# PRBonn/RAP

Measured on AMD Instinct MI355X. Metric: registered points/sec @20 flow steps, 2-view N=4096, higher is better.
Workload: dtype f32; 1 GPU; configs[1]: batch=32 samples/GPU x 2 views x 4096 pts, 20 Euler flow steps, rap_12 (d=512, H=8), fp32 (exact-fp32 MFMA), rigidity_forcing=on, final per-view SE(3) fit; preset=1, pairs_per_gpu=32, views=2, points_per_view=4096, flow_steps=20, num_layers=12, rigidity_forcing=True

## Files before the change

### rap_amd/csrc/api.hip

```cpp
#include "../../include/rapflow.h"
#include "half.h"
#include "kernels.h"

#include <mutex>
#include <new>
#include <vector>

static thread_local int g_last_hip_error = 0;
void rap_set_last_hip_error(int e) { g_last_hip_error = e; }

#define RAP_PROF_CLASSES 8
struct ProfRec { hipEvent_t a, b; int cls; };
static std::atomic<bool> g_prof_on{false};
static std::mutex g_prof_mu;
static std::vector<ProfRec> g_prof_recs;
static std::vector<hipEvent_t> g_prof_pool;
static size_t g_prof_pool_used = 0;
static const size_t RAP_PROF_MAX_EVENTS = 1u << 19;

static hipEvent_t prof_event() {
  if (g_prof_pool_used < g_prof_pool.size()) return g_prof_pool[g_prof_pool_used++];
  if (g_prof_pool.size() >= RAP_PROF_MAX_EVENTS) return nullptr;
  hipEvent_t e = nullptr;
  if (hipEventCreate(&e) != hipSuccess) return nullptr;
  g_prof_pool.push_back(e);
  g_prof_pool_used++;
  return e;
}
struct ProfScope {
  hipStream_t s; hipEvent_t a = nullptr, b = nullptr; int cls;
  ProfScope(hipStream_t s_, int cls_) : s(s_), cls(cls_) {
    if (!g_prof_on.load(std::memory_order_relaxed)) return;
    std::lock_guard<std::mutex> lock(g_prof_mu);
    a = prof_event(); b = prof_event();
    if (a && b) (void)hipEventRecord(a, s); else a = b = nullptr;
  }
  ~ProfScope() {
    if (a && b) {
      std::lock_guard<std::mutex> lock(g_prof_mu);
      (void)hipEventRecord(b, s); g_prof_recs.push_back({a, b, cls});
    }
  }
};
extern "C" int rap_profile_enable(int on) { g_prof_on.store(on != 0); return RAP_OK; }
extern "C" int rap_profile_reset(void) { std::lock_guard<std::mutex> lock(g_prof_mu); g_prof_recs.clear(); g_prof_pool_used = 0; return RAP_OK; }
extern "C" int rap_profile_collect_ex(float* h_ms_out, int64_t* h_count_out, int32_t n_classes) {
  if (!h_ms_out || !h_count_out || n_classes <= 0) return RAP_ERR_INVALID;
  std::lock_guard<std::mutex> lock(g_prof_mu);
  for (int c = 0; c < n_classes; ++c) { h_ms_out[c] = 0.f; h_count_out[c] = 0; }
  for (const ProfRec& r : g_prof_recs) {
    if (r.cls >= n_classes) continue;
    if (hipEventSynchronize(r.b) != hipSuccess) return RAP_ERR_HIP;
    float ms = 0.f;
    if (hipEventElapsedTime(&ms, r.a, r.b) != hipSuccess) return RAP_ERR_HIP;
    h_ms_out[r.cls] += ms; h_count_out[r.cls] += 1;
  }
  return RAP_OK;
}
extern "C" int rap_profile_collect(float* h_ms_out, int64_t* h_count_out) { return rap_profile_collect_ex(h_ms_out, h_count_out, 3); }

struct LayerW {
  const float* Wqkv[2];
  const float* Wout[2];
  const float* bout[2];
  const float* gq[2];
  const float* gk[2];
  const float* ffn_g;
  const float* ffn_b;
  const float* Wff1p;
  const float* bff1p;
  const float* Wff2;
  const float* bff2;
};

struct LayerWH {
  const u16* Wqkv[2];
  const u16* Wout[2];
  const u16* Wff1p;
  const u16* Wff2;
  float s_qkv[2] = {1.f, 1.f}, s_out[2] = {1.f, 1.f}, s_ff1 = 1.f, s_ff2 = 1.f;
  float g_v[2] = {1.f, 1.f}, g_ff1 = 1.f;
};
struct HalfWeights {
  u16* blob = nullptr;
  std::vector<LayerWH> layers;
};
#define RAP_MAX_LOGIT_BOUND 40.0f

struct rap_model {
  rap_model_desc desc;
  int d, L, H, F, E;
  int Din = 0;
  int Ks = 128;
  int dtype = RAP_DT_F32;
  bool qk_norm = true;
  int resid_dtype = RAP_DT_F32;
  HalfWeights half[4];
  float* logit_bound = nullptr;
  std::vector<uint8_t> bounded;
  int n_bounded = 0;
  float* raw = nullptr;
  float* derived = nullptr;
  const float* anchor_emb;
  const float* emb_bias;
  const float* Wstatic;
  const float* Wx;
  const float *adaW1, *adab1, *adaW2, *adab2, *adaW3, *adab3;
  std::vector<LayerW> layers;
  const float *hW0, *hb0, *hW2, *hb2, *hW4;
  mutable std::mutex cfg_mu;
};

static bool desc_ok(const rap_model_desc* d) {
  if (!d) return false;
  if (d->embed_dim <= 0 || d->embed_dim % 256 != 0 || d->embed_dim > 1024) return false;
  if (d->num_heads * 64 != d->embed_dim) return false;
  if (d->num_layers <= 0 || d->num_layers > 64) return false;
  if (d->local_feat_dim < 0 || d->local_feat_dim % 4 != 0 || d->local_feat_dim > 40) return false;
  return true;
}

extern rap_tuning_t g_rap_gemm_variant;
extern rap_tuning_t g_rap_gemm_stagger;
extern rap_tuning_t g_rap_gemm_splitk;
extern rap_tuning_t g_rap_geglu_fast;
extern rap_tuning_t g_rap_attn_split;
extern rap_tuning_t g_rap_gemm_h16_variant;
extern rap_tuning_t g_rap_attn_h16_variant;
extern rap_tuning_t g_rap_gemm_h16_persistent;
extern rap_tuning_t g_rap_attn_h16_dma;
extern rap_tuning_t g_rap_gemm_f32_persistent;
extern rap_tuning_t g_rap_attn_x2_wpe;
extern rap_tuning_t g_rap_attn_h16_small;
rap_tuning_t g_rap_attn_lpt = 1;
rap_tuning_t g_rap_x2_min_rows = 1024;
rap_tuning_t g_rap_small_fused = 1;
extern rap_tuning_t g_rap_ring_blocks;
rap_tuning_t g_rap_fuse_qknorm = 1;
struct TuningRow { int32_t key; rap_tuning_t* var; int n_values; int32_t values[7]; };
static const TuningRow kTuning[] = {
#ifdef RAP_ABLATION_BUILD
  {0, &g_rap_gemm_variant, 3, {16, 32, 48}},
  {2, &g_rap_gemm_h16_variant, 3, {0, 1, 14}},
  {3, &g_rap_attn_h16_variant, 2, {0, 5}},
  {4, &g_rap_gemm_stagger, 3, {0, 1, 2}},
#endif
  {5, &g_rap_attn_split, 2, {0, 1}},
  {6, &g_rap_gemm_splitk, 2, {0, 1}},
  {7, &g_rap_fuse_qknorm, 2, {0, 1}},
  {9, &g_rap_geglu_fast, 2, {0, 1}},
  {11, &g_rap_gemm_h16_persistent, 2, {0, 1}},
  {12, &g_rap_gemm_f32_persistent, 2, {0, 1}},
  {13, &g_rap_attn_h16_dma, 2, {0, 1}},
  {15, &g_rap_attn_lpt, 2, {0, 1}},
  {16, &g_rap_attn_x2_wpe, 2, {2, 4}},
  {17, &g_rap_x2_min_rows, -1, {}},
  {18, &g_rap_ring_blocks, -1, {}},
  {19, &g_rap_small_fused, 2, {0, 1}},
  {20, &g_rap_attn_h16_small, 7, {0, 1, 2, 64, 128, 66, 130}},
};
extern "C" int rap_set_tuning(int32_t key, int32_t value) {
  for (const TuningRow& r : kTuning) {
    if (r.key != key) continue;
    bool ok = r.n_values < 0 && value >= 0;
    for (int i = 0; i < r.n_values; ++i) ok = ok || r.values[i] == value;
    if (ok) *r.var = value;
    return ok ? RAP_OK : RAP_ERR_INVALID;
  }
  return RAP_ERR_INVALID;
}

extern "C" int rap_version(void) { return RAPFLOW_ABI_VERSION; }
extern "C" int rap_last_hip_error(void) { return g_last_hip_error; }

static bool in_dim_ok(int32_t in_dim) { return in_dim >= 0 && in_dim <= 512 && in_dim % 4 == 0; }
extern "C" int64_t rap_weight_count(const rap_model_desc* desc) { return rap_weight_count_latent(desc, 0); }
extern "C" int64_t rap_weight_count_latent(const rap_model_desc* desc, int32_t in_dim) {
  if (!desc_ok(desc) || !in_dim_ok(in_dim)) return -1;
  const int64_t d = desc->embed_dim, L = desc->num_layers, H = desc->num_heads, E = 147 + desc->local_feat_dim + in_dim;
  int64_t n = 2 * d + d * E + d;
  const int64_t attn = (d * 256 + d) + (d * d + d) + (2 * d * d + 2 * d) + 3 * d * d + (d * d + d) + 2 * H * 64;
  const int64_t layer = 2 * attn + 2 * d + (8 * d * d + 8 * d) + (4 * d * d + d);
  n += L * layer;
  n += (d * d + d) + (d / 2 * d + d / 2) + 3 * (d / 2);
  return n;
}

static int ensure_logit_bounds(rap_model* m, hipStream_t stream);

extern "C" int rap_model_create(const rap_model_desc* desc, const float* d_weights, int64_t n_floats, void* stream_,
                                rap_model** out) {
  return rap_model_create_latent(desc, 0, d_weights, n_floats, stream_, out);
}
extern "C" int rap_model_create_latent(const rap_model_desc* desc, int32_t in_dim, const float* d_weights, int64_t n_floats, void* stream_,
                                       rap_model** out) {
  if (!out) return RAP_ERR_INVALID;
  *out = nullptr;
  if (!desc_ok(desc) || !in_dim_ok(in_dim) || !d_weights) return RAP_ERR_INVALID;
  if (n_floats != rap_weight_count_latent(desc, in_dim)) return RAP_ERR_INVALID;
  hipStream_t stream = (hipStream_t)stream_;
  rap_model* m = new (std::nothrow) rap_model();
  if (!m) return RAP_ERR_ALLOC;
  m->desc = *desc;
  const int d = m->d = desc->embed_dim, L = m->L = desc->num_layers, H = m->H = desc->num_heads;
  m->F = desc->local_feat_dim;
  m->Din = in_dim;
  const int Ks = m->Ks = 128 + (in_dim + 31) / 32 * 32;
  const int E = m->E = 147 + m->F + m->Din;
  if (hipMalloc((void**)&m->raw, (size_t)n_floats * sizeof(float)) != hipSuccess) { delete m; return RAP_ERR_ALLOC; }
  const size_t n_ada = (size_t)2 * L * ((size_t)d * 256 + d + (size_t)d * d + d + (size_t)2 * d * d + 2 * d);
  const size_t n_ff1 = (size_t)L * ((size_t)8 * d * d + 8 * d);
  const size_t n_derived = (size_t)d * Ks + (size_t)d * 64 + n_ada + n_ff1;
  if (hipMalloc((void**)&m->derived, n_derived * sizeof(float)) != hipSuccess) {
    (void)hipFree(m->raw); delete m; return RAP_ERR_ALLOC;
  }
  int rc = RAP_OK;
  auto fail = [&](int code) { rap_model_destroy(m); return code; };
  if (hipMemcpyAsync(m->raw, d_weights, (size_t)n_floats * sizeof(float), hipMemcpyDeviceToDevice, stream) != hipSuccess)
    return fail(RAP_ERR_HIP);

  const float* p = m->raw;
  auto take = [&](size_t n) { const float* r = p; p += n; return r; };
  m->anchor_emb = take((size_t)2 * d);
  const float* embW = take((size_t)d * E);
  m->emb_bias = take(d);

  float* q = m->derived;
  auto carve = [&](size_t n) { float* r = q; q += n; return r; };
  float* Wstatic = carve((size_t)d * Ks);
  float* Wx = carve((size_t)d * 64);
  float* aW1 = carve((size_t)2 * L * d * 256); float* ab1 = carve((size_t)2 * L * d);
  float* aW2 = carve((size_t)2 * L * d * d);   float* ab2 = carve((size_t)2 * L * d);
  float* aW3 = carve((size_t)2 * L * 2 * d * d); float* ab3 = carve((size_t)2 * L * 2 * d);
  m->Wstatic = Wstatic; m->Wx = Wx;
  m->adaW1 = aW1; m->adab1 = ab1; m->adaW2 = aW2; m->adab2 = ab2; m->adaW3 = aW3; m->adab3 = ab3;

  if ((rc = launch_fill_zero(stream, Wstatic, (size_t)d * Ks))) return fail(rc);
  if ((rc = launch_fill_zero(stream, Wx, (size_t)d * 64))) return fail(rc);
  if ((rc = launch_copy_cols(stream, embW, E, 0, Wstatic, Ks, 0, d, 63))) return fail(rc);
  if ((rc = launch_copy_cols(stream, embW, E, 126, Wstatic, Ks, 63, d, 21))) return fail(rc);
  if ((rc = launch_copy_cols(stream, embW, E, 147, Wstatic, Ks, 84, d, m->F))) return fail(rc);
  if ((rc = launch_copy_cols(stream, embW, E, 147 + m->F, Wstatic, Ks, 128, d, m->Din))) return fail(rc);
  if ((rc = launch_copy_cols(stream, embW, E, 63, Wx, 64, 0, d, 63))) return fail(rc);

  m->layers.resize(L);
  for (int i = 0; i < L; ++i) {
    LayerW& lw = m->layers[i];
    for (int a = 0; a < 2; ++a) {
      const int j = 2 * i + a;
      const float* W1 = take((size_t)d * 256); const float* b1 = take(d);
      const float* W2 = take((size_t)d * d);   const float* b2 = take(d);
      const float* W3 = take((size_t)2 * d * d); const float* b3 = take((size_t)2 * d);
      if ((rc = launch_copy_cols(stream, W1, 256, 0, aW1 + (size_t)j * d * 256, 256, 0, d, 256))) return fail(rc);
      if ((rc = launch_copy_cols(stream, b1, d, 0, ab1 + (size_t)j * d, d, 0, 1, d))) return fail(rc);
      if ((rc = launch_copy_cols(stream, W2, d, 0, aW2 + (size_t)j * d * d, d, 0, d, d))) return fail(rc);
      if ((rc = launch_copy_cols(stream, b2, d, 0, ab2 + (size_t)j * d, d, 0, 1, d))) return fail(rc);
      if ((rc = launch_copy_cols(stream, W3, d, 0, aW3 + (size_t)j * 2 * d * d, d, 0, 2 * d, d))) return fail(rc);
      if ((rc = launch_copy_cols(stream, b3, 2 * d, 0, ab3 + (size_t)j * 2 * d, 2 * d, 0, 1, 2 * d))) return fail(rc);
      lw.Wqkv[a] = take((size_t)3 * d * d);
      lw.Wout[a] = take((size_t)d * d);
      lw.bout[a] = take(d);
      lw.gq[a] = take((size_t)H * 64);
      lw.gk[a] = take((size_t)H * 64);
    }
    lw.ffn_g = take(d);
    lw.ffn_b = take(d);
    const float* Wff1 = take((size_t)8 * d * d);
    const float* bff1 = take((size_t)8 * d);
    float* Wp = carve((size_t)8 * d * d);
    float* bp = carve((size_t)8 * d);
    if ((rc = launch_geglu_interleave(stream, Wff1, bff1, Wp, bp, 4 * d, d))) return fail(rc);
    lw.Wff1p = Wp; lw.bff1p = bp;
    lw.Wff2 = take((size_t)d * 4 * d);
    lw.bff2 = take(d);
  }
  m->hW0 = take((size_t)d * d); m->hb0 = take(d);
  m->hW2 = take((size_t)(d / 2) * d); m->hb2 = take(d / 2);
  m->hW4 = take((size_t)3 * (d / 2));
  if ((int64_t)(p - m->raw) != n_floats || (size_t)(q - m->derived) != n_derived) return fail(RAP_ERR_INVALID);
  if ((rc = ensure_logit_bounds(m, stream))) return fail(rc);
  *out = m;
  return RAP_OK;
}

extern "C" void rap_model_destroy(rap_model* m) {
  if (!m) return;
  if (m->raw) (void)hipFree(m->raw);
  if (m->derived) (void)hipFree(m->derived);
  for (int i = 0; i < 4; ++i)
    if (m->half[i].blob) (void)hipFree(m->half[i].blob);
  if (m->logit_bound) (void)hipFree(m->logit_bound);
  delete m;
}

static int ensure_logit_bounds(rap_model* m, hipStream_t stream) {
  if (m->logit_bound) return RAP_OK;
  const int n = m->L * 2 * m->H;
  if (hipMalloc((void**)&m->logit_bound, (size_t)n * sizeof(float)) != hipSuccess) { m->logit_bound = nullptr; return RAP_ERR_ALLOC; }
  for (int i = 0; i < m->L; ++i)
    for (int a = 0; a < 2; ++a) {
      const int rc = launch_qk_logit_bound(stream, m->layers[i].gq[a], m->layers[i].gk[a], m->H, m->logit_bound + (size_t)(2 * i + a) * m->H);
      if (rc) return rc;
    }
  std::vector<float> hb(n);
  RAP_HIP_CHECK(hipMemcpyAsync(hb.data(), m->logit_bound, (size_t)n * sizeof(float), hipMemcpyDeviceToHost, stream));
  RAP_HIP_CHECK(hipStreamSynchronize(stream));
  m->bounded.assign((size_t)2 * m->L, 1);
  for (int j = 0; j < 2 * m->L; ++j)
    for (int h = 0; h < m->H; ++h)
      if (!(hb[(size_t)j * m->H + h] <= RAP_MAX_LOGIT_BOUND)) m->bounded[j] = 0;
  m->n_bounded = 0;
  for (uint8_t b : m->bounded) m->n_bounded += b;
// ... 600 lines not shown
```

### rap_amd/csrc/attn_f32.hip

```cpp
#include "kernels.h"

#define AQ_WAVE 64
#define AKV 64
#define KLD 68
#define VLD 64
#define ATTN_FENCE __builtin_amdgcn_sched_barrier(0x406);

__device__ __forceinline__ float xhalf_max(float v) {
  const auto r = __builtin_amdgcn_permlane32_swap(__float_as_uint(v), __float_as_uint(v), false, false);
  return fmaxf(__uint_as_float(r[0]), __uint_as_float(r[1]));
}
__device__ __forceinline__ float xhalf_sum(float v) {
  const auto r = __builtin_amdgcn_permlane32_swap(__float_as_uint(v), __float_as_uint(v), false, false);
  return __uint_as_float(r[0]) + __uint_as_float(r[1]);
}

#define ATTN_DEFER_THR 11.5f
__device__ __forceinline__ float amax3(float a, float b, float c) {
  float r;
  asm("v_max3_f32 %0, %1, %2, %3" : "=v"(r) : "v"(a), "v"(b), "v"(c));
  return r;
}

template <int NW, bool BOUNDED, bool SPLIT = false>
__global__ __launch_bounds__(64 * NW, 2) void attention_f32_kernel(const float* __restrict__ qkv, float* __restrict__ out,
                                                                  int TP, int heads, const AttnWorkItem* __restrict__ items,
                                                                  const float* __restrict__ bound, float* __restrict__ part_o,
                                                                  float* __restrict__ part_l) {
  __shared__ __attribute__((aligned(16))) float smem[2 * AKV * KLD + 2 * AKV * VLD];
  float* Ks = smem;
  float* Vs = smem + 2 * AKV * KLD;

  const int head = blockIdx.x % heads;
  const AttnWorkItem it = items[blockIdx.x / heads];
  const int len = it.seg_len;
  if (len <= 0) return;
  const int tid = threadIdx.x;
  const int lane = tid & 63, wave = tid >> 6;
  const int hi = lane >> 5, l31 = lane & 31;

  const size_t plane = (size_t)heads * TP * 64;
  const float* Qg = qkv + ((size_t)head * TP + it.seg_start) * 64;
  const float* Kg = Qg + plane;
  const float* Vg = Qg + 2 * plane;

  const int qw0 = it.q0 + wave * AQ_WAVE;
  const bool wave_active = qw0 < len;
  if (NW == 8) {
    if (__builtin_amdgcn_readfirstlane(threadIdx.x) >= 256) __builtin_amdgcn_s_setprio(1);
  }

  const float qscale = 0.125f * 1.44269504088896340736f;
  float qf[2][32];
#pragma unroll
  for (int qt = 0; qt < 2; ++qt) {
    int q = qw0 + qt * 32 + l31;
    q = q < len ? q : len - 1;
    const float* qp = Qg + (size_t)q * 64 + 4 * hi;
#pragma unroll
    for (int g = 0; g < 8; ++g) {
      const float4 v = *reinterpret_cast<const float4*>(qp + 8 * g);
      qf[qt][g * 4 + 0] = v.x * qscale;
      qf[qt][g * 4 + 1] = v.y * qscale;
      qf[qt][g * 4 + 2] = v.z * qscale;
      qf[qt][g * 4 + 3] = v.w * qscale;
    }
  }

  f32x16 o[2][2];
#pragma unroll
  for (int a = 0; a < 2; ++a)
#pragma unroll
    for (int b = 0; b < 2; ++b)
#pragma unroll
      for (int r = 0; r < 16; ++r) o[a][b][r] = 0.f;
  const bool bound_ok = BOUNDED ? (bound[head] <= 40.0f) : true;
  float mrun[2] = {-1e30f, -1e30f};
  float lsum[2] = {0.f, 0.f};

  constexpr int RS = 4 * NW;
  const int srow = tid >> 4;
  const int sc4 = (tid & 15) * 4;
  float4 rk0, rk1, rk2, rk3, rv0, rv1, rv2, rv3;
  const int nkv = (len + AKV - 1) / AKV;
  int t_begin = 0, t_end = nkv;
  if (SPLIT) {
    t_begin = (int)((long)nkv * blockIdx.y / gridDim.y);
    t_end = (int)((long)nkv * (blockIdx.y + 1) / gridDim.y);
  }
  const int koff = srow * KLD + sc4;
  const int voff = srow * VLD + sc4;

#define ATTN_LOAD_ONE(T, I, RK, RV)                                          \
  {                                                                          \
    int key_ = (T) * AKV + srow + RS * (I);                                  \
    key_ = key_ < len ? key_ : len - 1;                                      \
    RK = *reinterpret_cast<const float4*>(Kg + (size_t)key_ * 64 + sc4);     \
    RV = *reinterpret_cast<const float4*>(Vg + (size_t)key_ * 64 + sc4);     \
  }
#define ATTN_LOAD_TILE(T)          \
  ATTN_LOAD_ONE(T, 0, rk0, rv0)    \
  ATTN_LOAD_ONE(T, 1, rk1, rv1)    \
  if constexpr (NW == 4) {         \
    ATTN_LOAD_ONE(T, 2, rk2, rv2)  \
    ATTN_LOAD_ONE(T, 3, rk3, rv3)  \
  }
#define ATTN_STORE_ONE(BUF, I, RK, RV)                                                            \
  *reinterpret_cast<float4*>(&Ks[(BUF) * (AKV * KLD) + koff + RS * (I) * KLD]) = RK;              \
  *reinterpret_cast<float4*>(&Vs[(BUF) * (AKV * VLD) + voff + RS * (I) * VLD]) = RV;
#define ATTN_STORE_TILE(BUF)           \
  ATTN_STORE_ONE(BUF, 0, rk0, rv0)     \
  ATTN_STORE_ONE(BUF, 1, rk1, rv1)     \
  if constexpr (NW == 4) {             \
    ATTN_STORE_ONE(BUF, 2, rk2, rv2)   \
    ATTN_STORE_ONE(BUF, 3, rk3, rv3)   \
  }

  ATTN_LOAD_TILE(t_begin)
  ATTN_STORE_TILE(0)
  __syncthreads();

  for (int t = t_begin; t < t_end; ++t) {
    const int cur = (t - t_begin) & 1;
    const bool more = (t + 1) < t_end;
    if (more) { ATTN_LOAD_TILE(t + 1) }

    if (wave_active) {
      const float* Kc = Ks + cur * (AKV * KLD);
      const float* Vc = Vs + cur * (AKV * VLD);
#pragma unroll
      for (int kt = 0; kt < 2; ++kt) {
        const int kbase = t * AKV + kt * 32;
        if (kbase >= len) break;
        f32x16 st[2];
#pragma unroll
        for (int r = 0; r < 16; ++r) { st[0][r] = 0.f; st[1][r] = 0.f; }
        const float* kp = Kc + (kt * 32 + l31) * KLD + 4 * hi;
        const float* vp = Vc + (kt * 32 + 4 * hi) * VLD + 2 * l31;
        float4 kf = *reinterpret_cast<const float4*>(kp);
        float2 vfa, vfb;
#pragma unroll
        for (int g = 0; g < 8; ++g) {
          float4 kn = kf;
          if (g < 7) kn = *reinterpret_cast<const float4*>(kp + 8 * (g + 1));
          else { vfa = *reinterpret_cast<const float2*>(vp); vfb = *reinterpret_cast<const float2*>(vp + VLD); }
          ATTN_FENCE
          st[0] = __builtin_amdgcn_mfma_f32_32x32x2f32(kf.x, qf[0][g * 4 + 0], st[0], 0, 0, 0);
          st[1] = __builtin_amdgcn_mfma_f32_32x32x2f32(kf.x, qf[1][g * 4 + 0], st[1], 0, 0, 0);
          st[0] = __builtin_amdgcn_mfma_f32_32x32x2f32(kf.y, qf[0][g * 4 + 1], st[0], 0, 0, 0);
          st[1] = __builtin_amdgcn_mfma_f32_32x32x2f32(kf.y, qf[1][g * 4 + 1], st[1], 0, 0, 0);
          st[0] = __builtin_amdgcn_mfma_f32_32x32x2f32(kf.z, qf[0][g * 4 + 2], st[0], 0, 0, 0);
          st[1] = __builtin_amdgcn_mfma_f32_32x32x2f32(kf.z, qf[1][g * 4 + 2], st[1], 0, 0, 0);
          st[0] = __builtin_amdgcn_mfma_f32_32x32x2f32(kf.w, qf[0][g * 4 + 3], st[0], 0, 0, 0);
          st[1] = __builtin_amdgcn_mfma_f32_32x32x2f32(kf.w, qf[1][g * 4 + 3], st[1], 0, 0, 0);
          ATTN_FENCE
          kf = kn;
        }
        if (kbase + 32 > len) {
#pragma unroll
          for (int r = 0; r < 16; ++r) {
            const bool valid = (kbase + mfma32_crow(r, hi)) < len;
            st[0][r] = valid ? st[0][r] : -1e30f;
            st[1][r] = valid ? st[1][r] : -1e30f;
          }
        }
        if (BOUNDED) {
#pragma unroll
          for (int qt = 0; qt < 2; ++qt) {
            float pa = 0.f, pb2 = 0.f;
#pragma unroll
            for (int r = 0; r < 16; r += 2) {
              const float e0 = __builtin_amdgcn_exp2f(st[qt][r]);
              const float e1 = __builtin_amdgcn_exp2f(st[qt][r + 1]);
              st[qt][r] = e0; st[qt][r + 1] = e1;
              pa += e0; pb2 += e1;
            }
            lsum[qt] += pa + pb2;
          }
        } else {
#pragma unroll
        for (int qt = 0; qt < 2; ++qt) {
          float mx = amax3(st[qt][0], st[qt][1], st[qt][2]);
#pragma unroll
          for (int r = 3; r < 15; r += 2) mx = amax3(mx, st[qt][r], st[qt][r + 1]);
          mx = xhalf_max(fmaxf(mx, st[qt][15]));
          if (__builtin_amdgcn_ballot_w64(mx > mrun[qt] + ATTN_DEFER_THR) != 0) {
            const float mnew = fmaxf(mrun[qt], mx);
            const float alpha = __builtin_amdgcn_exp2f(mrun[qt] - mnew);
            mrun[qt] = mnew;
            lsum[qt] *= alpha;
#pragma unroll
            for (int r = 0; r < 16; ++r) {
              o[qt][0][r] *= alpha;
              o[qt][1][r] *= alpha;
            }
          }
          float pa = 0.f, pb2 = 0.f;
#pragma unroll
          for (int r = 0; r < 16; r += 2) {
            const float e0 = __builtin_amdgcn_exp2f(st[qt][r] - mrun[qt]);
            const float e1 = __builtin_amdgcn_exp2f(st[qt][r + 1] - mrun[qt]);
            st[qt][r] = e0; st[qt][r + 1] = e1;
            pa += e0; pb2 += e1;
          }
          lsum[qt] += pa + pb2;
        }
        }
#pragma unroll
        for (int r = 0; r < 16; r += 2) {
          float2 vna = vfa, vnb = vfb;
          if (r + 2 < 16) {
            const int k0 = ((r + 2) & 3) + 8 * ((r + 2) >> 2);
            const int k1 = ((r + 3) & 3) + 8 * ((r + 3) >> 2);
            vna = *reinterpret_cast<const float2*>(vp + k0 * VLD);
            vnb = *reinterpret_cast<const float2*>(vp + k1 * VLD);
          }
          ATTN_FENCE
          o[0][0] = __builtin_amdgcn_mfma_f32_32x32x2f32(vfa.x, st[0][r], o[0][0], 0, 0, 0);
          o[0][1] = __builtin_amdgcn_mfma_f32_32x32x2f32(vfa.y, st[0][r], o[0][1], 0, 0, 0);
          o[1][0] = __builtin_amdgcn_mfma_f32_32x32x2f32(vfa.x, st[1][r], o[1][0], 0, 0, 0);
          o[1][1] = __builtin_amdgcn_mfma_f32_32x32x2f32(vfa.y, st[1][r], o[1][1], 0, 0, 0);
          o[0][0] = __builtin_amdgcn_mfma_f32_32x32x2f32(vfb.x, st[0][r + 1], o[0][0], 0, 0, 0);
          o[0][1] = __builtin_amdgcn_mfma_f32_32x32x2f32(vfb.y, st[0][r + 1], o[0][1], 0, 0, 0);
          o[1][0] = __builtin_amdgcn_mfma_f32_32x32x2f32(vfb.x, st[1][r + 1], o[1][0], 0, 0, 0);
          o[1][1] = __builtin_amdgcn_mfma_f32_32x32x2f32(vfb.y, st[1][r + 1], o[1][1], 0, 0, 0);
          ATTN_FENCE
          vfa = vna; vfb = vnb;
        }
      }
    }

    if (more) { ATTN_STORE_TILE(cur ^ 1) }
    __syncthreads();
  }

  if (!wave_active) return;
  const int dmodel = heads * 64;
#pragma unroll
  for (int qt = 0; qt < 2; ++qt) {
    const int q = qw0 + qt * 32 + l31;
    const float ltot = xhalf_sum(lsum[qt]);
    const float inv = SPLIT ? 1.0f : (bound_ok ? 1.0f / ltot : __builtin_nanf(""));
    if (q < len) {
      float* op = (SPLIT ? part_o + (size_t)blockIdx.y * TP * dmodel : out) + (size_t)(it.seg_start + q) * dmodel + head * 64;
      if (SPLIT && hi == 0)
        part_l[((size_t)blockIdx.y * TP + it.seg_start + q) * heads + head] = bound_ok ? ltot : __builtin_nanf("");
#pragma unroll
      for (int rg = 0; rg < 4; ++rg) {
        const int d0 = 2 * (8 * rg + 4 * hi);
        float4 w0, w1;
        w0.x = o[qt][0][4 * rg + 0] * inv; w0.y = o[qt][1][4 * rg + 0] * inv;
        w0.z = o[qt][0][4 * rg + 1] * inv; w0.w = o[qt][1][4 * rg + 1] * inv;
        w1.x = o[qt][0][4 * rg + 2] * inv; w1.y = o[qt][1][4 * rg + 2] * inv;
        w1.z = o[qt][0][4 * rg + 3] * inv; w1.w = o[qt][1][4 * rg + 3] * inv;
        *reinterpret_cast<float4*>(op + d0) = w0;
        *reinterpret_cast<float4*>(op + d0 + 4) = w1;
      }
    }
  }
}

#define WL_THREADS 1024
#define WL_TILE 4096
#define WL_SORT_MAX 8192
__device__ __forceinline__ int wl_len(const int32_t* __restrict__ cu, int s) { const int l = cu[s + 1] - cu[s]; return l > 0 ? l : 0; }
__global__ __launch_bounds__(WL_THREADS) void build_attn_worklist_kernel(const int32_t* __restrict__ cu, int nseg, AttnWorkItem* __restrict__ items,
                                                                          int max_items, int bq, int32_t* __restrict__ sort_ws) {
  if (blockIdx.x != 0) return;
  const int tid = threadIdx.x;
  const AttnWorkItem none = {0, 0, 0, 0};
  if (!sort_ws) {
    if (tid != 0) return;
    int n = 0;
    for (int s = 0; s < nseg; ++s) {
      const int a = cu[s], len = wl_len(cu, s);
      for (int q0 = 0; q0 < len && n < max_items; q0 += bq) { const AttnWorkItem w = {a, len, q0, 0}; items[n++] = w; }
    }
    for (; n < max_items; ++n) items[n] = none;
    return;
  }
  __shared__ int lens[WL_TILE];
  __shared__ int partial[WL_THREADS];
  __shared__ int total_items;
  int32_t* order = sort_ws;
  if (nseg > WL_SORT_MAX) {
    for (int s = tid; s < nseg; s += WL_THREADS) order[s] = s;
  } else
  for (int s0 = 0; s0 < nseg; s0 += WL_THREADS) {
    const int s = s0 + tid;
    const int my = s < nseg ? wl_len(cu, s) : -1;
    int rank = 0;
    for (int j0 = 0; j0 < nseg; j0 += WL_TILE) {
      __syncthreads();
      for (int j = tid; j < WL_TILE && j0 + j < nseg; j += WL_THREADS) lens[j] = wl_len(cu, j0 + j);
      __syncthreads();
      const int nj = nseg - j0 < WL_TILE ? nseg - j0 : WL_TILE;
      if (s < nseg)
        for (int j = 0; j < nj; ++j) rank += (lens[j] > my || (lens[j] == my && j0 + j < s)) ? 1 : 0;
    }
    if (s < nseg) order[rank] = s;
  }
  __threadfence_block();
  __syncthreads();
  const int per = (nseg + WL_THREADS - 1) / WL_THREADS;
  const int r0 = tid * per, r1 = (r0 + per) < nseg ? (r0 + per) : nseg;
  int sum = 0;
  for (int r = r0; r < r1; ++r) { const int sg = order[r]; sum += (wl_len(cu, sg) + bq - 1) / bq; }
  partial[tid] = sum;
  __syncthreads();
  if (tid == 0) {
    int acc = 0;
    for (int t = 0; t < WL_THREADS; ++t) { const int v = partial[t]; partial[t] = acc; acc += v; }
    total_items = acc;
  }
  __syncthreads();
  int n = partial[tid];
  for (int r = r0; r < r1; ++r) {
    const int sg = order[r];
    const int a = cu[sg], len = wl_len(cu, sg);
    for (int q0 = 0; q0 < len; q0 += bq, ++n)
      if (n < max_items) { const AttnWorkItem w = {a, len, q0, 0}; items[n] = w; }
  }
  __syncthreads();
  const int total = total_items < 0 ? 0 : total_items < max_items ? total_items : max_items;
  for (int i = total + tid; i < max_items; i += WL_THREADS) items[i] = none;
}

rap_tuning_t g_rap_attn_variant = 1;
rap_tuning_t g_rap_attn_split = 1;
static int attn_block_queries() { return RAP_ATTN_BQ; }

int launch_build_attn_worklist(hipStream_t stream, const int32_t* cu_seqlens, int nseg, AttnWorkItem* items,
                               int max_items, int block_queries, int32_t* sort_ws) {
  if (max_items <= 0) return RAP_OK;
  hipLaunchKernelGGL(build_attn_worklist_kernel, dim3(1), dim3(WL_THREADS), 0, stream, cu_seqlens, nseg, items, max_items,
                     block_queries > 0 ? block_queries : attn_block_queries(), sort_ws);
  RAP_LAUNCH_CHECK();
  return RAP_OK;
}

__global__ __launch_bounds__(256) void attention_combine_kernel(const float* __restrict__ part_o, const float* __restrict__ part_l,
                                                                float* __restrict__ out, int TP, int heads, int splits,
                                                                const int32_t* __restrict__ cover_cu, int cover_nseg) {
  const int dmodel = heads * 64;
  const long i = (long)blockIdx.x * 256 + threadIdx.x;
  if (i >= (long)TP * dmodel / 4) return;
  const long t = i / (dmodel / 4);
  const int c = (int)(i % (dmodel / 4)) * 4;
  if (cover_cu && (t < cover_cu[0] || t >= cover_cu[cover_nseg])) {
    *reinterpret_cast<float4*>(out + t * dmodel + c) = float4{0.f, 0.f, 0.f, 0.f};
    return;
  }
  float4 acc = {0.f, 0.f, 0.f, 0.f};
  float l = 0.f;
  for (int s = 0; s < splits; ++s) {
    const float4 v = *reinterpret_cast<const float4*>(part_o + ((size_t)s * TP + t) * dmodel + c);
    acc.x += v.x; acc.y += v.y; acc.z += v.z; acc.w += v.w;
    l += part_l[((size_t)s * TP + t) * heads + (c >> 6)];
  }
  const float inv = (l > 0.f || l != l) ? 1.0f / l : 0.f;
  acc.x *= inv; acc.y *= inv; acc.z *= inv; acc.w *= inv;
  *reinterpret_cast<float4*>(out + t * dmodel + c) = acc;
}

int attention_f32_splits(int max_items, int heads, bool bounded) {
  if (!bounded || g_rap_attn_split == 0) return 1;
  const long blocks = (long)max_items * heads;
  return blocks <= 160 ? 4 : blocks <= 320 ? 2 : 1;
}

int launch_attention_f32(hipStream_t stream, const float* qkv, float* out, int TP, int heads, const AttnWorkItem* items,
                         int max_items, const float* bound, float* part_o, float* part_l, int splits, const int32_t* cover_cu,
                         int cover_nseg) {
  if (max_items <= 0 || TP <= 0) return RAP_OK;
  if (heads <= 0) return RAP_ERR_INVALID;
  if (splits > 1) {
    if (!bound || !part_o || !part_l) return RAP_ERR_INVALID;
    unsigned dyn = 0;
    if ((long)max_items * heads * splits <= 384) {
      dyn = 16384;
      if (hipFuncSetAttribute(reinterpret_cast<const void*>(attention_f32_kernel<4, true, true>), hipFuncAttributeMaxDynamicSharedMemorySize, dyn) != hipSuccess) {
        rap_set_last_hip_error((int)hipGetLastError());
        return RAP_ERR_HIP;
      }
    }
    hipLaunchKernelGGL((attention_f32_kernel<4, true, true>), dim3(max_items * heads, splits), dim3(256), dyn, stream, qkv, out, TP,
                       heads, items, bound, part_o, part_l);
    RAP_LAUNCH_CHECK();
    const long n4 = (long)TP * heads * 16;
    hipLaunchKernelGGL(attention_combine_kernel, dim3((unsigned)((n4 + 255) / 256)), dim3(256), 0, stream, part_o, part_l, out, TP,
                       heads, splits, cover_cu, cover_nseg);
    RAP_LAUNCH_CHECK();
    return RAP_OK;
  }
  float* const no = nullptr;
  if (bound) hipLaunchKernelGGL((attention_f32_kernel<4, true>), dim3(max_items * heads), dim3(256), 0, stream, qkv, out, TP, heads, items, bound, no, no);
  else hipLaunchKernelGGL((attention_f32_kernel<4, false>), dim3(max_items * heads), dim3(256), 0, stream, qkv, out, TP, heads, items, bound, no, no);
  RAP_LAUNCH_CHECK();
  return RAP_OK;
}
```

Baseline: 16280 points/s.

## Add software-pipelined fp32 attention kernel overlapping LDS stores with PV MFMAs

Adds a PIPE variant of the fp32 flash-attention kernel, enabled by default through a new tuning key. It prefetches K/V tiles two iterations ahead and interleaves the shared-memory stores of the next tile with the PV MFMA loop of the second subtile. The last PV MFMAs are deferred past the barrier, and the first K fragment of the next tile is preloaded. Full tiles use unclamped direct-offset global loads. The aim is to hide barrier and LDS store latency behind MFMA work, at the cost of more register pressure and more complex control flow. An ablation-only timestamp probe is also added.

```diff
diff --git a/rap_amd/csrc/api.hip b/rap_amd/csrc/api.hip
--- a/rap_amd/csrc/api.hip
+++ b/rap_amd/csrc/api.hip
@@ -125,6 +125,7 @@
 extern rap_tuning_t g_rap_gemm_splitk;
 extern rap_tuning_t g_rap_geglu_fast;
 extern rap_tuning_t g_rap_attn_split;
+extern rap_tuning_t g_rap_attn_form;
 extern rap_tuning_t g_rap_gemm_h16_variant;
 extern rap_tuning_t g_rap_attn_h16_variant;
 extern rap_tuning_t g_rap_gemm_h16_persistent;
@@ -158,6 +159,7 @@
   {18, &g_rap_ring_blocks, -1, {}},
   {19, &g_rap_small_fused, 2, {0, 1}},
   {20, &g_rap_attn_h16_small, 7, {0, 1, 2, 64, 128, 66, 130}},
+  {22, &g_rap_attn_form, 2, {0, 1}},
 };
 extern "C" int rap_set_tuning(int32_t key, int32_t value) {
   for (const TuningRow& r : kTuning) {
diff --git a/rap_amd/csrc/attn_f32.hip b/rap_amd/csrc/attn_f32.hip
--- a/rap_amd/csrc/attn_f32.hip
+++ b/rap_amd/csrc/attn_f32.hip
@@ -1,4 +1,5 @@
 #include "kernels.h"
+#include <type_traits>
 
 #define AQ_WAVE 64
 #define AKV 64
@@ -22,11 +23,34 @@
   return r;
 }
 
-template <int NW, bool BOUNDED, bool SPLIT = false>
-__global__ __launch_bounds__(64 * NW, 2) void attention_f32_kernel(const float* __restrict__ qkv, float* __restrict__ out,
-                                                                  int TP, int heads, const AttnWorkItem* __restrict__ items,
-                                                                  const float* __restrict__ bound, float* __restrict__ part_o,
-                                                                  float* __restrict__ part_l) {
+#ifdef RAP_ABLATION_BUILD
+#define ATTN_TS_BLOCKS 1024
+#define ATTN_TS_TILES 64
+#define ATTN_TS_STRIDE (2 + 2 * ATTN_TS_TILES)
+__device__ unsigned long long* g_attn_ts = nullptr;
+extern "C" int rap_debug_attn_ts(void* p) { return hipMemcpyToSymbol(HIP_SYMBOL(g_attn_ts), &p, sizeof(p)) == hipSuccess ? 0 : -3; }
+#define ATTN_TS_ON (g_attn_ts && threadIdx.x == 0 && blockIdx.x < ATTN_TS_BLOCKS && blockIdx.y == 0)
+#define ATTN_TS_ENTRY                                                                                                    \
+  if (ATTN_TS_ON) {                                                                                                      \
+    g_attn_ts[(size_t)blockIdx.x * ATTN_TS_STRIDE] = __builtin_amdgcn_s_memrealtime();                                   \
+    g_attn_ts[(size_t)blockIdx.x * ATTN_TS_STRIDE + 1] =                                                                 \
+        ((unsigned long long)(__builtin_amdgcn_s_getreg((31 << 11) | 20) & 15u) << 16) | (__builtin_amdgcn_s_getreg((31 << 11) | 4) & 0xffffu); \
+  }
+#define ATTN_TS(TILE, I)                                                                                                 \
+  {                                                                                                                      \
+    __builtin_amdgcn_sched_barrier(0);                                                                                   \
+    if (ATTN_TS_ON && (TILE) >= 0 && (TILE) < ATTN_TS_TILES) g_attn_ts[(size_t)blockIdx.x * ATTN_TS_STRIDE + 2 + 2 * (TILE) + (I)] = __builtin_amdgcn_s_memtime(); \
+    __builtin_amdgcn_sched_barrier(0);                                                                                   \
+  }
+#else
+#define ATTN_TS_ENTRY
+#define ATTN_TS(TILE, I)
+#endif
+
+template <int NW, bool BOUNDED, bool SPLIT, bool PIPE>
+__device__ __forceinline__ void attention_f32_body(const float* __restrict__ qkv, float* __restrict__ out, int TP, int heads,
+                                                   const AttnWorkItem* __restrict__ items, const float* __restrict__ bound,
+                                                   float* __restrict__ part_o, float* __restrict__ part_l) {
   __shared__ __attribute__((aligned(16))) float smem[2 * AKV * KLD + 2 * AKV * VLD];
   float* Ks = smem;
   float* Vs = smem + 2 * AKV * KLD;
@@ -35,8 +59,10 @@
   const AttnWorkItem it = items[blockIdx.x / heads];
   const int len = it.seg_len;
   if (len <= 0) return;
+  ATTN_TS_ENTRY
   const int tid = threadIdx.x;
-  const int lane = tid & 63, wave = tid >> 6;
+  const int lane = tid & 63;
+  const int wave = PIPE ? __builtin_amdgcn_readfirstlane(tid >> 6) : tid >> 6;
   const int hi = lane >> 5, l31 = lane & 31;
 
   const size_t plane = (size_t)heads * TP * 64;
@@ -90,6 +116,7 @@
   }
   const int koff = srow * KLD + sc4;
   const int voff = srow * VLD + sc4;
+  const int goff = srow * 64 + sc4;
 
 #define ATTN_LOAD_ONE(T, I, RK, RV)                                          \
   {                                                                          \
@@ -98,12 +125,26 @@
     RK = *reinterpret_cast<const float4*>(Kg + (size_t)key_ * 64 + sc4);     \
     RV = *reinterpret_cast<const float4*>(Vg + (size_t)key_ * 64 + sc4);     \
   }
-#define ATTN_LOAD_TILE(T)          \
-  ATTN_LOAD_ONE(T, 0, rk0, rv0)    \
-  ATTN_LOAD_ONE(T, 1, rk1, rv1)    \
-  if constexpr (NW == 4) {         \
-    ATTN_LOAD_ONE(T, 2, rk2, rv2)  \
-    ATTN_LOAD_ONE(T, 3, rk3, rv3)  \
+#define ATTN_LOAD_FULL(I, RK, RV)                                            \
+  RK = *reinterpret_cast<const float4*>(Kt_ + goff + RS * 64 * (I));         \
+  RV = *reinterpret_cast<const float4*>(Vt_ + goff + RS * 64 * (I));
+#define ATTN_LOAD_TILE(T)                                 \
+  if (PIPE && ((T) + 1) * AKV <= len) {                   \
+    const float* Kt_ = Kg + (size_t)(T) * (AKV * 64);     \
+    const float* Vt_ = Vg + (size_t)(T) * (AKV * 64);     \
+    ATTN_LOAD_FULL(0, rk0, rv0)                           \
+    ATTN_LOAD_FULL(1, rk1, rv1)                           \
+    if constexpr (NW == 4) {                              \
+      ATTN_LOAD_FULL(2, rk2, rv2)                         \
+      ATTN_LOAD_FULL(3, rk3, rv3)                         \
+    }                                                     \
+  } else {                                                \
+    ATTN_LOAD_ONE(T, 0, rk0, rv0)                         \
+    ATTN_LOAD_ONE(T, 1, rk1, rv1)                         \
+    if constexpr (NW == 4) {                              \
+      ATTN_LOAD_ONE(T, 2, rk2, rv2)                       \
+      ATTN_LOAD_ONE(T, 3, rk3, rv3)                       \
+    }                                                     \
   }
 #define ATTN_STORE_ONE(BUF, I, RK, RV)                                                            \
   *reinterpret_cast<float4*>(&Ks[(BUF) * (AKV * KLD) + koff + RS * (I) * KLD]) = RK;              \
@@ -116,122 +157,189 @@
     ATTN_STORE_ONE(BUF, 3, rk3, rv3)   \
   }
 
+  float4 kf0 = {0.f, 0.f, 0.f, 0.f};
+  float hp[2][4] = {{0.f, 0.f, 0.f, 0.f}, {0.f, 0.f, 0.f, 0.f}};
+  float2 hv[4] = {{0.f, 0.f}, {0.f, 0.f}, {0.f, 0.f}, {0.f, 0.f}};
+
+  auto subtile = [&](auto kt_c, int t, int cur) __attribute__((always_inline)) {
+    constexpr int kt = decltype(kt_c)::value;
+    constexpr bool HOLD = PIPE && kt == 1;
+    const float* Kc = Ks + cur * (AKV * KLD);
+    const float* Vc = Vs + cur * (AKV * VLD);
+    const int kbase = t * AKV + kt * 32;
+    f32x16 st[2];
+#pragma unroll
+    for (int r = 0; r < 16; ++r) { st[0][r] = 0.f; st[1][r] = 0.f; }
+    const float* kp = Kc + (kt * 32 + l31) * KLD + 4 * hi;
+    const float* vp = Vc + (kt * 32 + 4 * hi) * VLD + 2 * l31;
+    float4 kf;
+    if constexpr (PIPE && kt == 0) kf = kf0;
+    else kf = *reinterpret_cast<const float4*>(kp);
+    float2 vfa, vfb;
+#pragma unroll
+    for (int g = 0; g < 8; ++g) {
+      float4 kn = kf;
+      if (g < 7) kn = *reinterpret_cast<const float4*>(kp + 8 * (g + 1));
+      else { vfa = *reinterpret_cast<const float2*>(vp); vfb = *reinterpret_cast<const float2*>(vp + VLD); }
+      ATTN_FENCE
+      st[0] = __builtin_amdgcn_mfma_f32_32x32x2f32(kf.x, qf[0][g * 4 + 0], st[0], 0, 0, 0);
+      st[1] = __builtin_amdgcn_mfma_f32_32x32x2f32(kf.x, qf[1][g * 4 + 0], st[1], 0, 0, 0);
+      st[0] = __builtin_amdgcn_mfma_f32_32x32x2f32(kf.y, qf[0][g * 4 + 1], st[0], 0, 0, 0);
+      st[1] = __builtin_amdgcn_mfma_f32_32x32x2f32(kf.y, qf[1][g * 4 + 1], st[1], 0, 0, 0);
+      st[0] = __builtin_amdgcn_mfma_f32_32x32x2f32(kf.z, qf[0][g * 4 + 2], st[0], 0, 0, 0);
+      st[1] = __builtin_amdgcn_mfma_f32_32x32x2f32(kf.z, qf[1][g * 4 + 2], st[1], 0, 0, 0);
+      st[0] = __builtin_amdgcn_mfma_f32_32x32x2f32(kf.w, qf[0][g * 4 + 3], st[0], 0, 0, 0);
+      st[1] = __builtin_amdgcn_mfma_f32_32x32x2f32(kf.w, qf[1][g * 4 + 3], st[1], 0, 0, 0);
+      ATTN_FENCE
+      kf = kn;
+    }
+    if (kbase + 32 > len) {
+#pragma unroll
+      for (int r = 0; r < 16; ++r) {
+        const bool valid = (kbase + mfma32_crow(r, hi)) < len;
+        st[0][r] = valid ? st[0][r] : -1e30f;
+        st[1][r] = valid ? st[1][r] : -1e30f;
+      }
+    }
+    if (BOUNDED) {
+#pragma unroll
+      for (int qt = 0; qt < 2; ++qt) {
+        float pa = 0.f, pb2 = 0.f;
+#pragma unroll
+        for (int r = 0; r < 16; r += 2) {
+          const float e0 = __builtin_amdgcn_exp2f(st[qt][r]);
+          const float e1 = __builtin_amdgcn_exp2f(st[qt][r + 1]);
+          st[qt][r] = e0; st[qt][r + 1] = e1;
+          pa += e0; pb2 += e1;
+        }
+        lsum[qt] += pa + pb2;
+      }
+    } else {
+#pragma unroll
+    for (int qt = 0; qt < 2; ++qt) {
+      float mx = amax3(st[qt][0], st[qt][1], st[qt][2]);
+#pragma unroll
+      for (int r = 3; r < 15; r += 2) mx = amax3(mx, st[qt][r], st[qt][r + 1]);
+      mx = xhalf_max(fmaxf(mx, st[qt][15]));
+      if (__builtin_amdgcn_ballot_w64(mx > mrun[qt] + ATTN_DEFER_THR) != 0) {
+        const float mnew = fmaxf(mrun[qt], mx);
+        const float alpha = __builtin_amdgcn_exp2f(mrun[qt] - mnew);
+        mrun[qt] = mnew;
+        lsum[qt] *= alpha;
+#pragma unroll
+        for (int r = 0; r < 16; ++r) {
+          o[qt][0][r] *= alpha;
+          o[qt][1][r] *= alpha;
+        }
+      }
+      float pa = 0.f, pb2 = 0.f;
+#pragma unroll
+      for (int r = 0; r < 16; r += 2) {
+        const float e0 = __builtin_amdgcn_exp2f(st[qt][r] - mrun[qt]);
+        const float e1 = __builtin_amdgcn_exp2f(st[qt][r + 1] - mrun[qt]);
+        st[qt][r] = e0; st[qt][r + 1] = e1;
+        pa += e0; pb2 += e1;
+      }
+      lsum[qt] += pa + pb2;
+    }
+    }
+    constexpr int R_END = HOLD ? 12 : 16;
+    float2 vha = {0.f, 0.f}, vhb = {0.f, 0.f};
+#pragma unroll
+    for (int r = 0; r < R_END; r += 2) {
+      float2 vna = vfa, vnb = vfb;
+      if (r + 2 < 16) {
+        const int k0 = ((r + 2) & 3) + 8 * ((r + 2) >> 2);
+        const int k1 = ((r + 3) & 3) + 8 * ((r + 3) >> 2);
+        vna = *reinterpret_cast<const float2*>(vp + k0 * VLD);
+        vnb = *reinterpret_cast<const float2*>(vp + k1 * VLD);
+      }
+      if constexpr (HOLD) {
+        if (r == 10) {
+          vha = *reinterpret_cast<const float2*>(vp + (2 + 8 * 3) * VLD);
+          vhb = *reinterpret_cast<const float2*>(vp + (3 + 8 * 3) * VLD);
+        }
+        if (r == 0) { ATTN_STORE_ONE(cur ^ 1, 0, rk0, rv0) }
+        if (r == 2) { ATTN_STORE_ONE(cur ^ 1, 1, rk1, rv1) }
+        if (NW == 4 && r == 4) { ATTN_STORE_ONE(cur ^ 1, 2, rk2, rv2) }
+        if (NW == 4 && r == 6) { ATTN_STORE_ONE(cur ^ 1, 3, rk3, rv3) }
+      }
+      ATTN_FENCE
+      o[0][0] = __builtin_amdgcn_mfma_f32_32x32x2f32(vfa.x, st[0][r], o[0][0], 0, 0, 0);
+      o[0][1] = __builtin_amdgcn_mfma_f32_32x32x2f32(vfa.y, st[0][r], o[0][1], 0, 0, 0);
+      o[1][0] = __builtin_amdgcn_mfma_f32_32x32x2f32(vfa.x, st[1][r], o[1][0], 0, 0, 0);
+      o[1][1] = __builtin_amdgcn_mfma_f32_32x32x2f32(vfa.y, st[1][r], o[1][1], 0, 0, 0);
+      o[0][0] = __builtin_amdgcn_mfma_f32_32x32x2f32(vfb.x, st[0][r + 1], o[0][0], 0, 0, 0);
+      o[0][1] = __builtin_amdgcn_mfma_f32_32x32x2f32(vfb.y, st[0][r + 1], o[0][1], 0, 0, 0);
+      o[1][0] = __builtin_amdgcn_mfma_f32_32x32x2f32(vfb.x, st[1][r + 1], o[1][0], 0, 0, 0);
+      o[1][1] = __builtin_amdgcn_mfma_f32_32x32x2f32(vfb.y, st[1][r + 1], o[1][1], 0, 0, 0);
+      ATTN_FENCE
+      vfa = vna; vfb = vnb;
+    }
+    if constexpr (HOLD) {
+      hv[0] = vfa; hv[1] = vfb; hv[2] = vha; hv[3] = vhb;
+#pragma unroll
+      for (int j = 0; j < 4; ++j) { hp[0][j] = st[0][12 + j]; hp[1][j] = st[1][12 + j]; }
+    }
+  };
+  const std::integral_constant<int, 0> KT0;
+  const std::integral_constant<int, 1> KT1;
+
   ATTN_LOAD_TILE(t_begin)
   ATTN_STORE_TILE(0)
+  if constexpr (PIPE) {
+    if (t_begin + 1 < t_end) { ATTN_LOAD_TILE(t_begin + 1) }
+  }
   __syncthreads();
 
-  for (int t = t_begin; t < t_end; ++t) {
-    const int cur = (t - t_begin) & 1;
-    const bool more = (t + 1) < t_end;
-    if (more) { ATTN_LOAD_TILE(t + 1) }
-
-    if (wave_active) {
-      const float* Kc = Ks + cur * (AKV * KLD);
-      const float* Vc = Vs + cur * (AKV * VLD);
-#pragma unroll
-      for (int kt = 0; kt < 2; ++kt) {
-        const int kbase = t * AKV + kt * 32;
-        if (kbase >= len) break;
-        f32x16 st[2];
-#pragma unroll
-        for (int r = 0; r < 16; ++r) { st[0][r] = 0.f; st[1][r] = 0.f; }
-        const float* kp = Kc + (kt * 32 + l31) * KLD + 4 * hi;
-        const float* vp = Vc + (kt * 32 + 4 * hi) * VLD + 2 * l31;
-        float4 kf = *reinterpret_cast<const float4*>(kp);
-        float2 vfa, vfb;
-#pragma unroll
-        for (int g = 0; g < 8; ++g) {
-          float4 kn = kf;
-          if (g < 7) kn = *reinterpret_cast<const float4*>(kp + 8 * (g + 1));
-          else { vfa = *reinterpret_cast<const float2*>(vp); vfb = *reinterpret_cast<const float2*>(vp + VLD); }
-          ATTN_FENCE
-          st[0] = __builtin_amdgcn_mfma_f32_32x32x2f32(kf.x, qf[0][g * 4 + 0], st[0], 0, 0, 0);
-          st[1] = __builtin_amdgcn_mfma_f32_32x32x2f32(kf.x, qf[1][g * 4 + 0], st[1], 0, 0, 0);
-          st[0] = __builtin_amdgcn_mfma_f32_32x32x2f32(kf.y, qf[0][g * 4 + 1], st[0], 0, 0, 0);
-          st[1] = __builtin_amdgcn_mfma_f32_32x32x2f32(kf.y, qf[1][g * 4 + 1], st[1], 0, 0, 0);
-          st[0] = __builtin_amdgcn_mfma_f32_32x32x2f32(kf.z, qf[0][g * 4 + 2], st[0], 0, 0, 0);
-          st[1] = __builtin_amdgcn_mfma_f32_32x32x2f32(kf.z, qf[1][g * 4 + 2], st[1], 0, 0, 0);
-          st[0] = __builtin_amdgcn_mfma_f32_32x32x2f32(kf.w, qf[0][g * 4 + 3], st[0], 0, 0, 0);
-          st[1] = __builtin_amdgcn_mfma_f32_32x32x2f32(kf.w, qf[1][g * 4 + 3], st[1], 0, 0, 0);
-          ATTN_FENCE
-          kf = kn;
+  if constexpr (!PIPE) {
+    for (int t = t_begin; t < t_end; ++t) {
+      const int cur = (t - t_begin) & 1;
+      const bool more = (t + 1) < t_end;
+      if (more) { ATTN_LOAD_TILE(t + 1) }
+      ATTN_TS(t - t_begin - 1, 1)
+      if (wave_active) {
+        subtile(KT0, t, cur);
+        if (t * AKV + 32 < len) subtile(KT1, t, cur);
+      }
+      ATTN_TS(t - t_begin, 0)
+      if (more) { ATTN_STORE_TILE(cur ^ 1) }
+      __syncthreads();
+    }
+  } else {
+    kf0 = *reinterpret_cast<const float4*>(Ks + l31 * KLD + 4 * hi);
+    for (int t = t_begin; t < t_end; ++t) {
+      const int cur = (t - t_begin) & 1;
+      const bool more = (t + 1) < t_end;
+      const bool second = wave_active && (t * AKV + 32 < len);
+      if (wave_active) {
+        subtile(KT0, t, cur);
+        if (second) subtile(KT1, t, cur);
+      }
+      if (more && !second) { ATTN_STORE_TILE(cur ^ 1) }
+      ATTN_TS(t - t_begin, 0)
+      __builtin_amdgcn_sched_barrier(0);
+      __syncthreads();
+      __builtin_amdgcn_sched_barrier(0);
+      ATTN_TS(t - t_begin, 1)
+      kf0 = *reinterpret_cast<const float4*>(Ks + (cur ^ 1) * (AKV * KLD) + l31 * KLD + 4 * hi);
+      if (second) {
+        ATTN_FENCE
+#pragma unroll
+        for (int j = 0; j < 4; j += 2) {
+          o[0][0] = __builtin_amdgcn_mfma_f32_32x32x2f32(hv[j].x, hp[0][j], o[0][0], 0, 0, 0);
+          o[0][1] = __builtin_amdgcn_mfma_f32_32x32x2f32(hv[j].y, hp[0][j], o[0][1], 0, 0, 0);
+          o[1][0] = __builtin_amdgcn_mfma_f32_32x32x2f32(hv[j].x, hp[1][j], o[1][0], 0, 0, 0);
+          o[1][1] = __builtin_amdgcn_mfma_f32_32x32x2f32(hv[j].y, hp[1][j], o[1][1], 0, 0, 0);
+          o[0][0] = __builtin_amdgcn_mfma_f32_32x32x2f32(hv[j + 1].x, hp[0][j + 1], o[0][0], 0, 0, 0);
+          o[0][1] = __builtin_amdgcn_mfma_f32_32x32x2f32(hv[j + 1].y, hp[0][j + 1], o[0][1], 0, 0, 0);
+          o[1][0] = __builtin_amdgcn_mfma_f32_32x32x2f32(hv[j + 1].x, hp[1][j + 1], o[1][0], 0, 0, 0);
+          o[1][1] = __builtin_amdgcn_mfma_f32_32x32x2f32(hv[j + 1].y, hp[1][j + 1], o[1][1], 0, 0, 0);
         }
-        if (kbase + 32 > len) {
-#pragma unroll
-          for (int r = 0; r < 16; ++r) {
-            const bool valid = (kbase + mfma32_crow(r, hi)) < len;
-            st[0][r] = valid ? st[0][r] : -1e30f;
-            st[1][r] = valid ? st[1][r] : -1e30f;
-          }
-        }
-        if (BOUNDED) {
-#pragma unroll
-          for (int qt = 0; qt < 2; ++qt) {
-            float pa = 0.f, pb2 = 0.f;
-#pragma unroll
-            for (int r = 0; r < 16; r += 2) {
-              const float e0 = __builtin_amdgcn_exp2f(st[qt][r]);
-              const float e1 = __builtin_amdgcn_exp2f(st[qt][r + 1]);
-              st[qt][r] = e0; st[qt][r + 1] = e1;
-              pa += e0; pb2 += e1;
-            }
-            lsum[qt] += pa + pb2;
-          }
-        } else {
-#pragma unroll
-        for (int qt = 0; qt < 2; ++qt) {
-          float mx = amax3(st[qt][0], st[qt][1], st[qt][2]);
-#pragma unroll
-          for (int r = 3; r < 15; r += 2) mx = amax3(mx, st[qt][r], st[qt][r + 1]);
-          mx = xhalf_max(fmaxf(mx, st[qt][15]));
-          if (__builtin_amdgcn_ballot_w64(mx > mrun[qt] + ATTN_DEFER_THR) != 0) {
-            const float mnew = fmaxf(mrun[qt], mx);
-            const float alpha = __builtin_amdgcn_exp2f(mrun[qt] - mnew);
-            mrun[qt] = mnew;
-            lsum[qt] *= alpha;
-#pragma unroll
-            for (int r = 0; r < 16; ++r) {
-              o[qt][0][r] *= alpha;
-              o[qt][1][r] *= alpha;
-            }
-          }
-          float pa = 0.f, pb2 = 0.f;
-#pragma unroll
-          for (int r = 0; r < 16; r += 2) {
-            const float e0 = __builtin_amdgcn_exp2f(st[qt][r] - mrun[qt]);
-            const float e1 = __builtin_amdgcn_exp2f(st[qt][r + 1] - mrun[qt]);
-            st[qt][r] = e0; st[qt][r + 1] = e1;
-            pa += e0; pb2 += e1;
-          }
-          lsum[qt] += pa + pb2;
-        }
-        }
-#pragma unroll
-        for (int r = 0; r < 16; r += 2) {
-          float2 vna = vfa, vnb = vfb;
-          if (r + 2 < 16) {
-            const int k0 = ((r + 2) & 3) + 8 * ((r + 2) >> 2);
-            const int k1 = ((r + 3) & 3) + 8 * ((r + 3) >> 2);
-            vna = *reinterpret_cast<const float2*>(vp + k0 * VLD);
-            vnb = *reinterpret_cast<const float2*>(vp + k1 * VLD);
-          }
-          ATTN_FENCE
-          o[0][0] = __builtin_amdgcn_mfma_f32_32x32x2f32(vfa.x, st[0][r], o[0][0], 0, 0, 0);
-          o[0][1] = __builtin_amdgcn_mfma_f32_32x32x2f32(vfa.y, st[0][r], o[0][1], 0, 0, 0);
-          o[1][0] = __builtin_amdgcn_mfma_f32_32x32x2f32(vfa.x, st[1][r], o[1][0], 0, 0, 0);
-          o[1][1] = __builtin_amdgcn_mfma_f32_32x32x2f32(vfa.y, st[1][r], o[1][1], 0, 0, 0);
-          o[0][0] = __builtin_amdgcn_mfma_f32_32x32x2f32(vfb.x, st[0][r + 1], o[0][0], 0, 0, 0);
-          o[0][1] = __builtin_amdgcn_mfma_f32_32x32x2f32(vfb.y, st[0][r + 1], o[0][1], 0, 0, 0);
-          o[1][0] = __builtin_amdgcn_mfma_f32_32x32x2f32(vfb.x, st[1][r + 1], o[1][0], 0, 0, 0);
-          o[1][1] = __builtin_amdgcn_mfma_f32_32x32x2f32(vfb.y, st[1][r + 1], o[1][1], 0, 0, 0);
-          ATTN_FENCE
-          vfa = vna; vfb = vnb;
-        }
-      }
-    }
-
-    if (more) { ATTN_STORE_TILE(cur ^ 1) }
-    __syncthreads();
+        ATTN_FENCE
+      }
+      if (t + 2 < t_end) { ATTN_LOAD_TILE(t + 2) }
+    }
   }
 
   if (!wave_active) return;
@@ -258,6 +366,21 @@
       }
     }
   }
+}
+
+template <int NW, bool BOUNDED, bool SPLIT = false>
+__global__ __launch_bounds__(64 * NW, 2) void attention_f32_kernel(const float* __restrict__ qkv, float* __restrict__ out,
+                                                                  int TP, int heads, const AttnWorkItem* __restrict__ items,
+                                                                  const float* __restrict__ bound, float* __restrict__ part_o,
+                                                                  float* __restrict__ part_l) {
+  attention_f32_body<NW, BOUNDED, SPLIT, false>(qkv, out, TP, heads, items, bound, part_o, part_l);
+}
+template <int NW, bool BOUNDED, bool SPLIT = false>
+__global__ __launch_bounds__(64 * NW, 2) void attention_f32_pipe_kernel(const float* __restrict__ qkv, float* __restrict__ out,
+                                                                       int TP, int heads, const AttnWorkItem* __restrict__ items,
+                                                                       const float* __restrict__ bound, float* __restrict__ part_o,
+                                                                       float* __restrict__ part_l) {
+  attention_f32_body<NW, BOUNDED, SPLIT, true>(qkv, out, TP, heads, items, bound, part_o, part_l);
 }
 
 #define WL_THREADS 1024
@@ -328,6 +451,7 @@
 
 rap_tuning_t g_rap_attn_variant = 1;
 rap_tuning_t g_rap_attn_split = 1;
+rap_tuning_t g_rap_attn_form = 1;
 static int attn_block_queries() { return RAP_ATTN_BQ; }
 
 int launch_build_attn_worklist(hipStream_t stream, const int32_t* cu_seqlens, int nseg, AttnWorkItem* items,
@@ -374,18 +498,22 @@
                          int cover_nseg) {
   if (max_items <= 0 || TP <= 0) return RAP_OK;
   if (heads <= 0) return RAP_ERR_INVALID;
+  const bool pipe = g_rap_attn_form != 0;
   if (splits > 1) {
     if (!bound || !part_o || !part_l) return RAP_ERR_INVALID;
     unsigned dyn = 0;
     if ((long)max_items * heads * splits <= 384) {
       dyn = 16384;
-      if (hipFuncSetAttribute(reinterpret_cast<const void*>(attention_f32_kernel<4, true, true>), hipFuncAttributeMaxDynamicSharedMemorySize, dyn) != hipSuccess) {
+      const void* fn = pipe ? reinterpret_cast<const void*>(attention_f32_pipe_kernel<4, true, true>) : reinterpret_cast<const void*>(attention_f32_kernel<4, true, true>);
+      if (hipFuncSetAttribute(fn, hipFuncAttributeMaxDynamicSharedMemorySize, dyn) != hipSuccess) {
         rap_set_last_hip_error((int)hipGetLastError());
         return RAP_ERR_HIP;
       }
     }
-    hipLaunchKernelGGL((attention_f32_kernel<4, true, true>), dim3(max_items * heads, splits), dim3(256), dyn, stream, qkv, out, TP,
-                       heads, items, bound, part_o, part_l);
+    if (pipe) hipLaunchKernelGGL((attention_f32_pipe_kernel<4, true, true>), dim3(max_items * heads, splits), dim3(256), dyn, stream, qkv, out, TP,
+                                 heads, items, bound, part_o, part_l);
+    else hipLaunchKernelGGL((attention_f32_kernel<4, true, true>), dim3(max_items * heads, splits), dim3(256), dyn, stream, qkv, out, TP,
+                            heads, items, bound, part_o, part_l);
     RAP_LAUNCH_CHECK();
     const long n4 = (long)TP * heads * 16;
     hipLaunchKernelGGL(attention_combine_kernel, dim3((unsigned)((n4 + 255) / 256)), dim3(256), 0, stream, part_o, part_l, out, TP,
@@ -394,8 +522,14 @@
     return RAP_OK;
   }
   float* const no = nullptr;
-  if (bound) hipLaunchKernelGGL((attention_f32_kernel<4, true>), dim3(max_items * heads), dim3(256), 0, stream, qkv, out, TP, heads, items, bound, no, no);
-  else hipLaunchKernelGGL((attention_f32_kernel<4, false>), dim3(max_items * heads), dim3(256), 0, stream, qkv, out, TP, heads, items, bound, no, no);
+  const dim3 grid(max_items * heads);
+  if (pipe) {
+    if (bound) hipLaunchKernelGGL((attention_f32_pipe_kernel<4, true>), grid, dim3(256), 0, stream, qkv, out, TP, heads, items, bound, no, no);
+    else hipLaunchKernelGGL((attention_f32_pipe_kernel<4, false>), grid, dim3(256), 0, stream, qkv, out, TP, heads, items, bound, no, no);
+  } else {
+    if (bound) hipLaunchKernelGGL((attention_f32_kernel<4, true>), grid, dim3(256), 0, stream, qkv, out, TP, heads, items, bound, no, no);
+    else hipLaunchKernelGGL((attention_f32_kernel<4, false>), grid, dim3(256), 0, stream, qkv, out, TP, heads, items, bound, no, no);
+  }
   RAP_LAUNCH_CHECK();
   return RAP_OK;
 }
```

Result: no change. 16360 points/s (median of 6 runs) (+0.5%).
